# chriscoey/Hypatia.jl

Hardware: AMD Instinct MI355X
Metric: IPM iterations/sec (+ ms per KKT solve): dense n=5000, PosSemidefTri side 200 (Float64, QRCholDense + CombinedStepper) (higher is better)
Workload: dtype f64

## Files before the change

### hypatia.jl_amd/csrc/directions_multi.hip

```cpp
#include <cstring>
#include "syssolver.hpp"
#include <chrono>

namespace hyp {

void seg_dots(Ctx& c, int B, int len, const double* a, const double* b, int off, int stride, double* out);
constexpr int MR = 2;

template <int NR, int TPB, int U>
__global__ __launch_bounds__(TPB) void gemv_t_multi_kernel(int m, double alpha, const double* __restrict__ A, long lda,
                                                           const double* __restrict__ X, long ldx, double beta, double* __restrict__ Y,
                                                           long ldy) {
  constexpr int NW = TPB / 64;
  __shared__ double red[NR][NW];
  const int col = blockIdx.x;
  const double* a = A + (long)col * lda;
  double s[NR][2 * U];
#pragma unroll
  for (int r = 0; r < NR; ++r)
#pragma unroll
    for (int u = 0; u < 2 * U; ++u) s[r][u] = 0.0;
  int i = 0;
  typedef double d2_t __attribute__((ext_vector_type(2)));
  const bool wide = (((uintptr_t)a | (uintptr_t)X | ((uintptr_t)ldx * sizeof(double))) & 15) == 0;
// ... 654 lines not shown
  } else {
    for (int r = 0; r < nr; ++r) tri_solves(sol + r * ld3);
  }
  gemv_multi(ctx, false, q, n, nr, 1.0, G.d(), q, sol, ld3, 0.0, m_Gx.d(), q);
  for (size_t k = 0; k < cones.size(); ++k) {
    Cone* ck = cones[k];
    if (const int used = run_hess_prod(k, m_HGx.d() + offs[k], q, m_Gx.d() + offs[k], q, nr)) { k += used - 1; continue; }
    if (ck->use_dual_barrier) ck->inv_hess_prod(m_HGx.d() + offs[k], q, m_Gx.d() + offs[k], q, nr);
    else ck->hess_prod(m_HGx.d() + offs[k], q, m_Gx.d() + offs[k], q, nr);
  }
  {
    LinK k{};
    for (int r = 0; r < nr; ++r) { k.k0[r] = 1.0; k.k1[r] = -1.0; }
    lincomb_cols(ctx, q, nr, m_HGx.d(), q, sol + n, ld3, nullptr, 0, sol + n, ld3, k);
  }
}

void SysSolver::get_directions2(double* h_dirs, const double* h_rhss, double mu, double taubar, int max_ref_steps, double res_norm_cutoff,
                                double min_impr_tol, double* res_norms, int* n_solves) {
  HYP_REQUIRE(model_loaded, "sys: load_model first");
  const size_t d = sizeof(double);
  const int dv = dimv(), it = n + p + q, ik = dv - 1;
  *n_solves = 0;
  if (p > 0) {
    for (int r = 0; r < MR; ++r) {
      int ns = 0;
      res_norms[r] = get_directions(h_dirs + (long)r * dv, h_rhss + (long)r * dv, mu, taubar, max_ref_steps, res_norm_cutoff, min_impr_tol, &ns);
      *n_solves += ns;
    }
    return;
  }
  m_rhs.ensure((size_t)MR * dv * d);
  double* rhs = m_rhs.d();
  ctx.h2d(rhs, h_rhss, (size_t)MR * dv * d);
  Scal rs[MR], dsc[MR];
  for (int r = 0; r < MR; ++r) {
    ctx.zero(rhs + (long)r * dv + it, d);
    ctx.zero(rhs + (long)r * dv + ik, d);
    rs[r] = Scal{h_rhss[(long)r * dv + it], h_rhss[(long)r * dv + ik]};
  }
  pair_solve_device(rhs, rs, mu, taubar, max_ref_steps, res_norm_cutoff, min_impr_tol, dsc, res_norms, n_solves);
  ctx.d2h(h_dirs, m_dir.d(), (size_t)MR * dv * d);
  ctx.sync();
  for (int r = 0; r < MR; ++r) {
    h_dirs[(long)r * dv + it] = dsc[r].tau;
    h_dirs[(long)r * dv + ik] = dsc[r].kap;
  }
}

struct TauArgs { double rs_tau[2], rs_kap[2], base_tau[2], base_kap[2]; double mu, taubar, dot_const, seq; int nr, const_mode, base_on, hz_sep; };
__global__ void cols_tau_kernel(double* __restrict__ sc, TauArgs a) {
#pragma clang fp contract(off)
  if (threadIdx.x != 0) return;
  double dc = a.dot_const;
  if (a.const_mode) dc = sc[SysSolver::SC_SOLVE + 4] + (a.hz_sep ? sc[SysSolver::SC_HZ + 2] : sc[SysSolver::SC_SOLVE + 5]);
  sc[SysSolver::SC_DOTC] = dc;
  const double m2 = a.mu / a.taubar / a.taubar;
  for (int r = 0; r < a.nr; ++r) {
    const double dot_sub = sc[SysSolver::SC_SOLVE + 2 * r] + (a.hz_sep ? sc[SysSolver::SC_HZ + r] : sc[SysSolver::SC_SOLVE + 2 * r + 1]);
    const double sol_tau = (a.rs_tau[r] + a.rs_kap[r] + dot_sub) / (m2 - dc);
    const double sol_kap = -a.mu / a.taubar / a.taubar * sol_tau + a.rs_kap[r];
    sc[SysSolver::SC_CSC + 2 * r] = sol_tau;
    sc[SysSolver::SC_CSC + 2 * r + 1] = sol_kap;
    sc[SysSolver::SC_DSC + 2 * r] = a.base_on ? a.base_tau[r] - sol_tau : sol_tau;
    sc[SysSolver::SC_DSC + 2 * r + 1] = a.base_on ? a.base_kap[r] - sol_kap : sol_kap;
  }
}

struct GemvOneGuard {
  Ctx& c;
  bool keep;
  GemvOneGuard(Ctx& ctx, bool on) : c(ctx), keep(ctx.gemv_one) { if (on) c.gemv_one = true; }
  ~GemvOneGuard() { c.gemv_one = keep; }
};

void SysSolver::ensure_d_sc() {
  if (d_sc.bytes >= SC_TOTAL * sizeof(double)) return;
  d_sc.alloc(SC_TOTAL * sizeof(double));
  ctx.zero(d_sc.p, SC_TOTAL * sizeof(double));
}

static bool dir_poll_on() {
  static const bool on = [] { const char* e = getenv("HYP_DIR_POLL"); return !(e && e[0] == '0'); }();
  return on;
}

bool SysSolver::dirs_resident() const {
  static const bool on = [] { const char* e = getenv("HYP_DIR_RESIDENT"); return !(e && e[0] == '0'); }();
  static const bool dist_on = [] { const char* e = getenv("HYP_DIST_RESIDENT"); return !(e && e[0] == '0'); }();
  return on && p == 0 && (!dist() || (dist_on && fused_ok()));
}

void SysSolver::cols_solve(double* sol, const double* rhs, int nr, const Scal* rs, double mu, double taubar, bool with_const, bool joint_const,
                           bool resident, bool both, const Scal* base, Scal* dsc_host) {
  const size_t d = sizeof(double);
  const int dv = dimv();
  HYP_REQUIRE(p == 0 && nr >= 1 && nr <= MR, "cols_solve: p = 0, one or two columns");
  HYP_REQUIRE(!(with_const || joint_const) || nr == MR, "cols_solve: the constant column rides with a pair");
  const int oz = n, os = n + q + 1;
  const long ld3 = n + q;
  for (DBuf* b : {&m_subr, &m_subs}) b->ensure((size_t)(MR + 1) * ld3 * d);
  for (DBuf* b : {&m_Gx, &m_HGx, &m_Gxd}) b->ensure((size_t)(MR + 1) * q * d);
  ensure_d_sc();
  double* sr = m_subr.d();
  double* ss = m_subs.d();
  double* sc = d_sc.d();
  const int ncol = with_const ? nr + 1 : nr;
  if (with_const) {
    double* rc = const_cast<double*>(rhs) + (long)MR * dv;
    ctx.zero(rc, (size_t)dv * d);
    dev_scale_copy(ctx, n, -1.0, mc.d(), rc);
    dev_scale_copy(ctx, q, -1.0, mh.d(), rc + oz);
  }
  for (int r = 0; r < ncol; ++r) ctx.d2d(sr + r * ld3, rhs + (long)r * dv, (size_t)n * d);
  LinK neg2{};
  for (int r = 0; r < MR + 1; ++r) { neg2.k0[r] = -1.0; neg2.k1[r] = -1.0; }
  for (size_t k = 0; k < cones.size(); ++k) {
    Cone* ck = cones[k];
    const int o = offs[k], dk = ck->dim;
    if (ck->use_dual_barrier) {
      for (int r = 0; r < ncol; ++r) {
        double* tmp = ss + r * ld3 + oz + o;
        dev_scale_copy(ctx, dk, -1.0, rhs + (long)r * dv + oz + o, tmp);
        dev_axpby(ctx, dk, -1.0, rhs + (long)r * dv + os + o, 1.0, tmp);
      }
      ck->inv_hess_prod(sr + oz + o, ld3, ss + oz + o, ld3, ncol);
    } else if (const int used = run_hess_prod(k, sr + oz + o, ld3, rhs + oz + o, dv, ncol)) {
      lincomb_cols(ctx, offs[k + used] - o, ncol, sr + oz + o, ld3, rhs + os + o, dv, nullptr, 0, sr + oz + o, ld3, neg2);
      k += used - 1;
    } else {
      ck->hess_prod(sr + oz + o, ld3, rhs + oz + o, dv, ncol);
      lincomb_cols(ctx, dk, ncol, sr + oz + o, ld3, rhs + os + o, dv, nullptr, 0, sr + oz + o, ld3, neg2);
    }
  }
  {
    GemvOneGuard g1(ctx, ncol == 1);
    solve3_multi(ss, sr, ncol, joint_const ? sol_const.d() : nullptr);
  }
  const bool dist_res = resident && dist();
  {
    DotSpecs sp;
    for (int r = 0; r < ncol; ++r) {
      sp.add(n, mc.d(), ss + r * ld3, sc + SC_SOLVE + 2 * r);
      sp.add(q, mh.d(), ss + r * ld3 + oz, dist_res ? sc + SC_HZ + r : sc + SC_SOLVE + 2 * r + 1);
    }
    if (joint_const) {
      update_const_post();
      sp.add(n, mc.d(), sol_const.d(), sc + SC_SOLVE + 2 * MR);
      sp.add(q, mh.d(), sol_const.d() + n, sc + SC_SOLVE + 2 * MR + 1);
    }
    dev_dots(ctx, sp);
  }
  if (dist_res) allreduce_dev(sc + SC_HZ, ncol, 0, 2);
  const bool own_const = with_const || joint_const;
  LinK k{};
  if (resident) {
    TauArgs a{};
    for (int r = 0; r < nr; ++r) {
      a.rs_tau[r] = rs[r].tau; a.rs_kap[r] = rs[r].kap;
      if (base) { a.base_tau[r] = base[r].tau; a.base_kap[r] = base[r].kap; }
    }
    a.mu = mu; a.taubar = taubar; a.dot_const = dot_const; a.nr = nr; a.const_mode = own_const ? 1 : 0; a.base_on = base ? 1 : 0;
    a.seq = (double)(++sc_seq);
    a.hz_sep = dist_res ? 1 : 0;
    hipLaunchKernelGGL(cols_tau_kernel, dim3(1), dim3(64), 0, ctx.stream, sc, a);
    HYP_CHECK(hipGetLastError());
// ... 305 lines not shown
  double* dir = m_dir.d();
  double* res = m_res.d();
  {
    ZeroSlots z;
    for (int r = 0; r < MR; ++r) {
      z.add(dir + (long)r * dv + it); z.add(dir + (long)r * dv + ik);
      z.add(res + (long)r * dv + it); z.add(res + (long)r * dv + ik);
    }
    dev_zero_slots(ctx, z);
  }
  const bool both = (max_ref_steps > 0) && gemv_both_ok(q, n, G.d(), q);
  cols_solve(dir, rhs, MR, rs, mu, taubar, with_const, joint_const, resident, both, nullptr, dsc_host);
  if (max_ref_steps > 0) cols_residual(res, dir, rhs, MR, dsc_host, resident, false, both);
  if (read_scalars) cols_read_scalars(resident);
}

void SysSolver::pair_finish(double* rhs, const Scal* rs, double mu, double taubar, int max_ref_steps, double res_norm_cutoff,
                            double min_impr_tol, bool with_const, bool joint_const, bool resident, Scal* dsc, double* res_norms, int* n_solves) {
  const size_t d = sizeof(double);
  const int dv = dimv();
  double* dir = m_dir.d();
  double* res = m_res.d();
  const double* hp = ctx.h_sc();
  if (resident && (with_const || joint_const)) dot_const = hp[SC_DOTC];
  *n_solves += MR;
  Scal rsc[MR];
  if (max_ref_steps <= 0) {
    for (int r = 0; r < MR; ++r) {
      if (resident) dsc[r] = Scal{hp[SC_DSC + 2 * r], hp[SC_DSC + 2 * r + 1]};
      res_norms[r] = 0.0;
    }
    return;
  }
  cols_finish(MR, rs, mu, taubar, resident, dsc, rsc, res_norms);
  Gx_dir_valid = false;
  if (!(res_norms[0] > res_norm_cutoff) && !(res_norms[1] > res_norm_cutoff)) return;
  bool cones_ok = true;
  for (const Cone* ck : cones) cones_ok = cones_ok && ck->products_columnwise();
  static const bool paired = [] { const char* e = getenv("HYP_REFINE_PAIRED"); return !(e && e[0] == '0'); }();
  if (paired && cones_ok && (!dist() || resident)) {
    refine_cols(rhs, dir, res, rs, dsc, rsc, res_norms, mu, taubar, max_ref_steps, res_norm_cutoff, min_impr_tol, n_solves, resident);
    return;
  }
  for (int r = 0; r < MR; ++r) {
    if (!(res_norms[r] > res_norm_cutoff)) continue;
    double* tmp = v_tmp.d();
    ctx.d2d(tmp, dir + (long)r * dv, (size_t)dv * d);
    res_norms[r] = refine(rhs + (long)r * dv, dir + (long)r * dv, res + (long)r * dv, tmp, rs[r], dsc[r], rsc[r], res_norms[r], mu, taubar,
                          max_ref_steps, res_norm_cutoff, min_impr_tol, n_solves);
  }
}

void SysSolver::pair_solve_device(double* rhs, const Scal* rs, double mu, double taubar, int max_ref_steps, double res_norm_cutoff,
                                  double min_impr_tol, Scal* dsc, double* res_norms, int* n_solves, bool with_const, bool joint_const) {
  const bool resident = dirs_resident();
  pair_enqueue(rhs, rs, mu, taubar, max_ref_steps, with_const, joint_const, resident, dsc);
  ctx.sync();
  pair_finish(rhs, rs, mu, taubar, max_ref_steps, res_norm_cutoff, min_impr_tol, with_const, joint_const, resident, dsc, res_norms, n_solves);
}


__global__ void dder3_gate_kernel(int dk, const double* __restrict__ dots, double irtrtmu, double rteps, const double* __restrict__ D3c,
                                  const double* __restrict__ Hqp, const double* __restrict__ D3p, double* __restrict__ c0, double* __restrict__ c1) {
#pragma clang fp contract(off)
  const int k = blockIdx.y;
  const int i = blockIdx.x * blockDim.x + threadIdx.x;
  if (i >= dk) return;
  const double* dd = dots + 4 * k;
  const long e = (long)k * dk + i;
  {
    const double dot1 = dd[0], dot2 = dd[1];
    if (fabs(dot1 - dot2) / (rteps + fabs(dot2)) < 1e-4) c0[e] = D3c[e];
  }
  {
    const double dot1 = dd[2], dot2 = irtrtmu * dd[3];
    if (fabs(dot1 - dot2) / (rteps + fabs(dot2)) < 1e-4) c1[e] = Hqp[e] + D3p[e];
  }
}

void SysSolver::build_rhs_pair(int stage, double* rhs2, const double* pt, double mu, double tau, double kap, double tau_residual,
                               const double* dirs2, const double* dir_tau2, double* rs_flat, bool resident) {
  const size_t d = sizeof(double);
  const int dv = dimv(), oz = n + p, os = n + p + q + 1;
  ctx.zero(rhs2, (size_t)MR * dv * d);
  double* c0 = rhs2;
  double* c1 = rhs2 + dv;
  Scal* rs = reinterpret_cast<Scal*>(rs_flat);
  if (stage == 0) {
    const double rtmu = std::sqrt(mu);
    ctx.d2d(c1, s_resid.d(), (size_t)n * d);
    ctx.d2d(c1 + oz, s_resid.d() + n + p, (size_t)q * d);
    if (const PsdRun* r = whole_model_run()) {
      run_g.ensure((size_t)q * d);
      run_grad(*r, run_g.d());
      dev_scale_copy(ctx, q, -1.0, pt + oz, c0 + os);
      dev_axpby(ctx, q, -rtmu, run_g.d(), 1.0, c0 + os);
      dev_scale_copy(ctx, q, -1.0, pt + oz, c1 + os);
      rs[0] = Scal{0.0, -kap + mu / tau};
      rs[1] = Scal{tau_residual, -kap};
      return;
    }
    for (size_t k = 0; k < cones.size(); ++k) {
      Cone* ck = cones[k];
      const int o = offs[k], dk = ck->dim;
      const double* dual = pt + (ck->use_dual_barrier ? os : oz) + o;
      dev_scale_copy(ctx, dk, -1.0, dual, c0 + os + o);
      dev_axpby(ctx, dk, -rtmu, ck->get_grad(), 1.0, c0 + os + o);
      dev_scale_copy(ctx, dk, -1.0, dual, c1 + os + o);
    }
    rs[0] = Scal{0.0, -kap + mu / tau};
    rs[1] = Scal{tau_residual, -kap};
    return;
  }
  const double rteps = std::sqrt(2.220446049250313e-16);
  const double irtrtmu = 1.0 / std::sqrt(std::sqrt(mu));
  for (DBuf* b : {&m_Gx, &m_HGx, &m_Gxd}) b->ensure((size_t)MR * q * d);
  double* scal = m_Gx.d();
  double* Hq = m_HGx.d();
  double* D3 = m_Gxd.d();
  const size_t nc = cones.size();
  s_dots.ensure(std::max<size_t>(4 * nc, 4) * d);
  double* dots = s_dots.d();
  const PsdRun* wr = whole_model_run();
  if (wr) {
    for (int r = 0; r < MR; ++r) {
      const double* prim = dirs2 + (long)r * dv + os;
      dev_scale_copy(ctx, q, irtrtmu, prim, scal + (long)r * q);
      const int used = run_hess_prod(0, Hq + (long)r * q, q, r == 0 ? scal : prim, q, 1);
      HYP_REQUIRE(used == (int)nc, "build_rhs_pair: run product");
      run_dder3(*wr, scal + (long)r * q, D3 + (long)r * q);
      seg_dots(ctx, (int)nc, cones[0]->dim, D3 + (long)r * q, wr->point, 2 * r, 4, dots);
      seg_dots(ctx, (int)nc, cones[0]->dim, scal + (long)r * q, Hq + (long)r * q, 2 * r + 1, 4, dots);
    }
  }
  static const bool d3_paired = [] { const char* e = getenv("HYP_DDER3_PAIRED"); return !(e && e[0] == '0'); }();
  std::vector<char> done_k(nc, 0);
  for (size_t k = 0; k < nc && !wr && d3_paired; ++k) {
    PsdCone* pk = dynamic_cast<PsdCone*>(cones[k]);
    if (!pk || !pk->use_dder3() || MR != 2) continue;
    const int o = offs[k], dk = pk->dim;
    const int po = (pk->use_dual_barrier ? oz : os) + o;
    m_subs.ensure((size_t)(MR + 1) * (n + q) * d);
    double* Hin = m_subs.d();
    LinK ks{}, kh{};
    for (int r = 0; r < MR; ++r) { ks.k0[r] = irtrtmu; kh.k0[r] = (r == 0) ? irtrtmu : 1.0; }
    lincomb_cols(ctx, dk, MR, dirs2 + po, dv, nullptr, 0, nullptr, 0, scal + o, q, ks);
    lincomb_cols(ctx, dk, MR, dirs2 + po, dv, nullptr, 0, nullptr, 0, Hin, dk, kh);
    pk->hess_prod_slow(Hq + o, q, Hin, dk, MR);
    pk->dder3_cols(scal + o, q, MR, D3 + o, q);
    done_k[k] = 1;
  }
  for (size_t k = 0; k < nc && !wr; ++k) {
    Cone* ck = cones[k];
    if (!ck->use_dder3() || done_k[k]) continue;
    const int o = offs[k], dk = ck->dim;
    const int po = (ck->use_dual_barrier ? oz : os) + o;
    for (int r = 0; r < MR; ++r) {
      const double* prim = dirs2 + (long)r * dv + po;
      double* sc = scal + (long)r * q + o;
      double* hh = Hq + (long)r * q + o;
      dev_scale_copy(ctx, dk, irtrtmu, prim, sc);
      ck->hess_prod_slow(hh, q, r == 0 ? sc : prim, q, 1);
      const double* d3 = ck->dder3(sc);
      ctx.d2d(D3 + (long)r * q + o, d3, (size_t)dk * d);
    }
  }
  for (size_t k = 0; k < nc && !wr; ++k) {
    Cone* ck = cones[k];
    if (!ck->use_dder3()) continue;
    const int o = offs[k], dk = ck->dim;
    if (d3_paired) {
      DotSpecs sp;
      for (int r = 0; r < MR; ++r) {
        sp.add(dk, D3 + (long)r * q + o, ck->point.d(), dots + 4 * k + 2 * r);
        sp.add(dk, scal + (long)r * q + o, Hq + (long)r * q + o, dots + 4 * k + 2 * r + 1);
      }
      dev_dots(ctx, sp);
      continue;
    }
    for (int r = 0; r < MR; ++r) {
      dev_dot(ctx, dk, D3 + (long)r * q + o, ck->point.d(), dots + 4 * k + 2 * r);
      dev_dot(ctx, dk, scal + (long)r * q + o, Hq + (long)r * q + o, dots + 4 * k + 2 * r + 1);
    }
  }
  const double tc = dir_tau2[0] / tau, tp = dir_tau2[1] / tau;
  rs[0] = Scal{0.0, tc * mu / tau * tc};
  rs[1] = Scal{0.0, tp * mu / tau * (1.0 + tp)};
  if (resident) {
    if (wr) {
      const int dk = cones[0]->dim;
      hipLaunchKernelGGL(dder3_gate_kernel, dim3((dk + 255) / 256, (unsigned)nc), dim3(256), 0, ctx.stream, dk, dots, irtrtmu, rteps, D3, Hq + q,
                         D3 + q, c0 + os, c1 + os);
    } else {
      for (size_t k = 0; k < nc; ++k) {
        Cone* ck = cones[k];
        if (!ck->use_dder3()) continue;
        const int o = offs[k], dk = ck->dim;
        hipLaunchKernelGGL(dder3_gate_kernel, dim3((dk + 255) / 256, 1), dim3(256), 0, ctx.stream, dk, dots + 4 * k, irtrtmu, rteps, D3 + o,
                           Hq + q + o, D3 + q + o, c0 + os + o, c1 + os + o);
      }
    }
    HYP_CHECK(hipGetLastError());
    return;
  }
  std::vector<double> hd(4 * std::max<size_t>(nc, 1));
  ctx.d2h(hd.data(), dots, 4 * nc * d);
  ctx.sync();
  for (size_t k = 0; k < nc; ++k) {
    Cone* ck = cones[k];
    if (!ck->use_dder3()) continue;
    const int o = offs[k], dk = ck->dim;
    {
      const double dot1 = hd[4 * k], dot2 = hd[4 * k + 1];
      if (std::fabs(dot1 - dot2) / (rteps + std::fabs(dot2)) < 1e-4) ctx.d2d(c0 + os + o, D3 + o, (size_t)dk * d);
    }
    {
      const double dot1 = hd[4 * k + 2], dot2 = irtrtmu * hd[4 * k + 3];
      if (std::fabs(dot1 - dot2) / (rteps + std::fabs(dot2)) < 1e-4) {
        ctx.d2d(c1 + os + o, Hq + q + o, (size_t)dk * d);
        dev_axpby(ctx, dk, 1.0, D3 + q + o, 1.0, c1 + os + o);
      }
    }
  }
}

void SysSolver::step_directions(const double* h_point, const double* h_res, double tau_residual, double mu, int max_ref_steps,
                                double res_norm_cutoff, double min_impr_tol, double* h_dirs, double* res_norms, int* n_solves,
                                int* use_sqrt_out, int* info, int* used_fallback, double* h_sol_const) {
  HYP_REQUIRE(model_loaded, "sys: load_model first");
  HYP_REQUIRE(p == 0, "step_directions: p = 0 only");
  const size_t d = sizeof(double);
  const int dv = dimv(), it = n + p + q, ik = dv - 1;
  *n_solves = 0;
  *info = 0;
  *used_fallback = 0;
  s_resident = false;
  double* hs_point = ctx.stage_host((size_t)dv + 2 * (size_t)it + 2 * (size_t)MR * dv);
  double* hs_res = hs_point + dv;
  double* hs_const = hs_res + it;
  double* hs_dirs = hs_const + it;
  s_point.ensure((size_t)dv * d);
  s_resid.ensure((size_t)it * d);
  auto upload = [&](hipStream_t st) {
    std::memcpy(hs_point, h_point, (size_t)dv * d);
    std::memcpy(hs_res, h_res, (size_t)it * d);
    HYP_CHECK(hipMemcpyAsync(s_point.p, hs_point, (size_t)dv * d, hipMemcpyHostToDevice, st));
    HYP_CHECK(hipMemcpyAsync(s_resid.p, hs_res, (size_t)it * d, hipMemcpyHostToDevice, st));
  };
  const bool resident_flow = dirs_resident() && nmp > 0 && !getenv_on("HYP_FORCE_BK") && !getenv_on("HYP_FORCE_FACT_FAIL");
  static const bool late_upload = [] { const char* e = getenv("HYP_LATE_UPLOAD"); return !(e && e[0] == '0'); }();
  const bool upload_late = resident_flow && late_upload && ctx.stream == ctx.stream_primary && (size_t)dv * d >= (1u << 20);
  if (upload_late) {
    if (!up_ev0) {
      HYP_CHECK(hipEventCreateWithFlags(&up_ev0, hipEventDisableTiming));
      HYP_CHECK(hipEventCreateWithFlags(&up_ev1, hipEventDisableTiming));
    }
    HYP_CHECK(hipEventRecord(up_ev0, ctx.stream));
  }
  static const bool after_env = [] { const char* e = getenv("HYP_UPLOAD_AFTER"); return !(e && e[0] == '0'); }();
  const bool upload_after = resident_flow && !upload_late && after_env;
  if (!upload_late && !upload_after) upload(ctx.stream);
  const auto t0 = std::chrono::steady_clock::now();
  const double tau = h_point[it], kap = h_point[ik];
  m_rhs.ensure((size_t)(MR + 1) * dv * d);
  v_tmp.ensure((size_t)MR * dv * d);
  const bool resident = resident_flow;
  if (!resident) {
    if (nmp > 0) update_lhs_fact(info, used_fallback);
    if (use_sqrt_out)
      for (size_t k = 0; k < cones.size(); ++k) use_sqrt_out[k] = use_sqrt[k];
    if (*info != 0) { ctx.sync(); return; }
    step_directions_rest(false, tau, kap, tau_residual, mu, max_ref_steps, res_norm_cutoff, min_impr_tol, h_dirs, res_norms, n_solves,
                         h_sol_const, hs_const, hs_dirs, false, nullptr, nullptr);
    last_update_lhs_s = last_rest_update_lhs_s + std::chrono::duration<double>(t_rest0 - t0).count();
    return;
  }
  assemble_lhs();
  factor_lhs_begin();
  if (upload_after) {
    hs_point = ctx.stage_host((size_t)dv + 2 * (size_t)it + 2 * (size_t)MR * dv);
    hs_res = hs_point + dv;
    hs_const = hs_res + it;
    hs_dirs = hs_const + it;
    upload(ctx.stream);
  }
  if (upload_late) {
    hs_point = ctx.stage_host((size_t)dv + 2 * (size_t)it + 2 * (size_t)MR * dv);
    hs_res = hs_point + dv;
    hs_const = hs_res + it;
    hs_dirs = hs_const + it;
    HYP_CHECK(hipStreamWaitEvent(ctx.stream2, up_ev0, 0));
    upload(ctx.stream2);
    HYP_CHECK(hipEventRecord(up_ev1, ctx.stream2));
    HYP_CHECK(hipStreamWaitEvent(ctx.stream, up_ev1, 0));
  }
  if (use_sqrt_out)
    for (size_t k = 0; k < cones.size(); ++k) use_sqrt_out[k] = use_sqrt[k];
  bool cones_ok = true;
  for (const Cone* ck : cones) cones_ok = cones_ok && ck->products_columnwise();
  const bool const3 = const3_on() && cones_ok;
  const bool joint = !const3 && tri3_on() && !dist() && tri.ready(nmp) && tri.sb > 0 && tri.sb <= 1024;
  if (!const3 && !joint) {
    update_const();
    if (h_sol_const) ctx.d2h(hs_const, sol_const.p, (size_t)it * d);
  }
  if (joint) update_const_pre();
  HYP_CHECK(hipEventRecord(ctx.ev[5], ctx.stream));
  Scal rs[MR], dsc[MR];
  double rn[MR];
  int ns = 0;
  build_rhs_pair(0, m_rhs.d(), s_point.d(), mu, tau, kap, tau_residual, nullptr, nullptr, reinterpret_cast<double*>(rs), true);
  pair_enqueue(m_rhs.d(), rs, mu, tau, max_ref_steps, const3, joint, true, dsc);
  wait_scalars();
  if (dir_poll_on() && ctx.h_sc_dev != nullptr) ctx.h_info[Ctx::H_INFO_FACT] = (int)ctx.h_sc()[SC_INFO];
  const auto tf0 = std::chrono::steady_clock::now();
  factor_lhs_end(info, used_fallback, true);
  const double fallback_s = std::chrono::duration<double>(std::chrono::steady_clock::now() - tf0).count();
  auto read_times = [&] {
    factor_lhs_times();
    float ms = 0;
    HYP_CHECK(hipEventElapsedTime(&ms, ctx.ev[0], ctx.ev[5]));
    last_update_lhs_s = 1e-3 * ms;
  };
  if (*info != 0 || use_bk) read_times();
  if (*info != 0) return;
  if (use_bk) {
    const double dev_s = last_update_lhs_s;
    step_directions_rest(false, tau, kap, tau_residual, mu, max_ref_steps, res_norm_cutoff, min_impr_tol, h_dirs, res_norms, n_solves,
                         h_sol_const, hs_const, hs_dirs, false, nullptr, nullptr);
    last_update_lhs_s = dev_s + fallback_s + last_rest_update_lhs_s;
    return;
  }
  pair_finish(m_rhs.d(), rs, mu, tau, max_ref_steps, res_norm_cutoff, min_impr_tol, const3, joint, true, dsc, rn, &ns);
  if ((const3 || joint) && h_sol_const) ctx.d2h(hs_const, sol_const.p, (size_t)it * d);
  *n_solves += ns;
  step_directions_rest(true, tau, kap, tau_residual, mu, max_ref_steps, res_norm_cutoff, min_impr_tol, h_dirs, res_norms, n_solves, h_sol_const,
                       hs_const, hs_dirs, true, dsc, rn);
  read_times();
}

static bool env_default_on(const char* name) {
  const char* e = getenv(name);
  return !(e && e[0] == '0');
}
bool SysSolver::const3_on() { static const bool on = env_default_on("HYP_CONST_COL3"); return on; }
bool SysSolver::tri3_on() { static const bool on = env_default_on("HYP_CONST_TRI3"); return on; }
bool SysSolver::getenv_on(const char* name) {
  const char* e = getenv(name);
  return e && e[0] && e[0] != '0';
}

void SysSolver::step_directions_rest(bool resident, double tau, double kap, double tau_residual, double mu, int max_ref_steps,
                                     double res_norm_cutoff, double min_impr_tol, double* h_dirs, double* res_norms, int* n_solves,
                                     double* h_sol_const, double* hs_const, double* hs_dirs, bool first_pair_done, Scal* d01_in, double* rn01) {
  const size_t d = sizeof(double);
  const int dv = dimv(), it = n + p + q, ik = dv - 1;
  t_rest0 = std::chrono::steady_clock::now();
  last_rest_update_lhs_s = 0.0;
  Scal rs[MR], dsc[MR];
  double rn[MR];
  int ns = 0;
  if (!first_pair_done) {
    bool cones_ok = true;
    for (const Cone* ck : cones) cones_ok = cones_ok && ck->products_columnwise();
    const bool const3 = const3_on() && !use_bk && cones_ok;
    const bool joint = !const3 && tri3_on() && !dist() && !use_bk && nmp > 0 && tri.ready(nmp) && tri.sb > 0 && tri.sb <= 1024;
    if (!const3 && !joint) {
      update_const();
      if (h_sol_const) ctx.d2h(hs_const, sol_const.p, (size_t)it * d);
    }
    if (joint) update_const_pre();
    last_rest_update_lhs_s = std::chrono::duration<double>(std::chrono::steady_clock::now() - t_rest0).count();
    build_rhs_pair(0, m_rhs.d(), s_point.d(), mu, tau, kap, tau_residual, nullptr, nullptr, reinterpret_cast<double*>(rs), resident);
    pair_enqueue(m_rhs.d(), rs, mu, tau, max_ref_steps, const3, joint, resident, dsc);
    ctx.sync();
    pair_finish(m_rhs.d(), rs, mu, tau, max_ref_steps, res_norm_cutoff, min_impr_tol, const3, joint, resident, dsc, rn, &ns);
    if ((const3 || joint) && h_sol_const) ctx.d2h(hs_const, sol_const.p, (size_t)it * d);
    *n_solves += ns;
  } else {
    dsc[0] = d01_in[0]; dsc[1] = d01_in[1];
    rn[0] = rn01[0]; rn[1] = rn01[1];
  }
  res_norms[0] = rn[0];
  res_norms[1] = rn[1];
  s_dirs.ensure((size_t)2 * MR * dv * d);
  const double dtau[MR] = {dsc[0].tau, dsc[1].tau};
  const Scal d01[MR] = {dsc[0], dsc[1]};
  build_rhs_pair(1, m_rhs.d(), s_point.d(), mu, tau, kap, tau_residual, m_dir.d(), dtau, reinterpret_cast<double*>(rs), resident);
  const size_t rows_down = dirs_x_only ? (size_t)n : (size_t)dv;
  auto dirs_d2h = [&](int half) {
    double* dst = hs_dirs + (long)half * MR * dv;
    if (!dirs_x_only) { ctx.d2h(dst, m_dir.d(), (size_t)MR * dv * d); return; }
    HYP_CHECK(hipMemcpy2DAsync(dst, (size_t)dv * d, m_dir.d(), (size_t)dv * d, rows_down * d, MR, hipMemcpyDeviceToHost, ctx.stream));
  };
  auto dirs_out = [&](int half) {
    for (int r = 0; r < MR; ++r)
      std::memcpy(h_dirs + ((long)half * MR + r) * dv, hs_dirs + ((long)half * MR + r) * dv, rows_down * d);
  };
  dirs_d2h(0);
  ctx.d2d(s_dirs.p, m_dir.p, (size_t)MR * dv * d);
  if (!dirs_copied_ev) HYP_CHECK(hipEventCreateWithFlags(&dirs_copied_ev, hipEventDisableTiming));
  HYP_CHECK(hipEventRecord(dirs_copied_ev, ctx.stream));
  ns = 0;
  pair_enqueue(m_rhs.d(), rs, mu, tau, max_ref_steps, false, false, resident, dsc, false);
  dirs_d2h(1);
  ctx.d2d(s_dirs.d() + (long)MR * dv, m_dir.p, (size_t)MR * dv * d);
  cols_read_scalars(resident);
  HYP_CHECK(hipEventSynchronize(dirs_copied_ev));
  dirs_out(0);
  if (resident) wait_scalars();
  else ctx.sync();
  const int ns_before = ns;
  pair_finish(m_rhs.d(), rs, mu, tau, max_ref_steps, res_norm_cutoff, min_impr_tol, false, false, resident, dsc, rn, &ns);
  *n_solves += ns;
  res_norms[2] = rn[0];
  res_norms[3] = rn[1];
  if (ns > ns_before + MR) {
    dirs_d2h(1);
    ctx.d2d(s_dirs.d() + (long)MR * dv, m_dir.p, (size_t)MR * dv * d);
    ctx.sync();
  }
  dirs_out(1);
  if (h_sol_const) std::memcpy(h_sol_const, hs_const, (size_t)it * d);
  for (int r = 0; r < MR; ++r) {
    h_dirs[(long)r * dv + it] = d01[r].tau;
    h_dirs[(long)r * dv + ik] = d01[r].kap;
    h_dirs[(long)(MR + r) * dv + it] = dsc[r].tau;
    h_dirs[(long)(MR + r) * dv + ik] = dsc[r].kap;
    s_tk[1 + r][0] = d01[r].tau;
    s_tk[1 + r][1] = d01[r].kap;
    s_tk[1 + MR + r][0] = dsc[r].tau;
    s_tk[1 + MR + r][1] = dsc[r].kap;
  }
  s_tk[0][0] = tau;
  s_tk[0][1] = kap;
  s_resident_q = q;
  s_resident = (MR == 2);
}

}
```

### hypatia.jl_amd/csrc/syssolver.hpp

```cpp
#pragma once
#include <chrono>
#include "cones.hpp"

namespace hyp {

void dev_sub_absmax(Ctx& c, int n, double* a, const double* b, double* d_out);
void dev_sub_absmax_cols(Ctx& c, int n, int nr, double* a, const double* b, long ld, double* d_out, double* work);

struct SysSolver {
  Ctx& ctx;
  int n, p, q, nmp;
  std::vector<Cone*> cones;
  std::vector<int> offs;
  DBuf G;
  DBuf GQ1;
  DBuf GQ2s;
  DBuf Qm;
  DBuf Rinv;
  DBuf HGQ2;
  DBuf lhs;
  DBuf lhs_tri;
  DBuf lhs_fact, dinv, d_info;
  TriSolvePlan tri;
  DBuf QpbxGHbz, Gx, HGx, GQ1x, HGQ1x, tmpn, sol, rhs, tmpq;
// ... 77 lines not shown
  void allreduce_fused(double* d_buf, long npay, const FusedTail& t, double* h_out, int site);
  void allreduce_fused_dev(double* d_buf, long npay, const FusedTail& t, int site);
  double screen_sz_[18];
  double screen_szfail_[18];
  int screen_pass_g_ = -1;
  DBuf rp_x, rp_z, rp_s, rp_t, rp_g;
  DBuf rp_loc;
  void prefetch_residual_products(int mode, double alpha, const double* d_cand, const double* h_cand);
  bool rp_pre_valid = false;
  double* rp_pre_host = nullptr;
  size_t rp_pre_host_n = 0;
  hipEvent_t rp_pre_ev = nullptr;
  std::vector<double> rp_pre_cand;
  long rp_pre_hits = 0, rp_pre_misses = 0;
  void residual_products2(const double* h_x, const double* h_z, const double* h_s, double tau, double* h_Gtz, double* h_Gx_s, double* h_dots,
                          double* h_norms);
  void residual_products(const double* h_x, const double* h_z, const double* h_s, double* h_Gtz, double* h_Gx_s, double* h_dots);

  DBuf mc, mb, mh, mA;
  DBuf v_rhs, v_dir, v_res, v_tmp;
  DBuf sub_rhs, sub_sol, sol_const;
  bool model_loaded = false;
  double dot_const = 0.0;
  DBuf Gx_dir;
  bool Gx_dir_valid = false;
  int dimv() const { return n + p + q + 1 + q + 1; }
  void load_model(const double* hc, const double* hb, const double* hh, const double* hA);
  void sgemv(bool trans, int m, int n_, double alpha, const double* A, long lda, const double* x, double beta, double* y);
  void update_const();
  void update_const_pre();
  void update_const_post();
  struct Scal { double tau, kap; };
  Scal solve_system(double* d_sol, const double* d_rhs, Scal rhs, double mu, double taubar);
  Scal apply_lhs(double* d_res, const double* d_dir, Scal dir, double mu, double taubar);
  DBuf cand_d;
  bool check_cone_points(const double* h_ztsk, double min_prox, double prox_bound, bool use_max_prox, double nup1, double* prox_out,
                         int* n_loaded, double* irtmu_out);
  static constexpr int SCREEN_MAX = 18;
  DBuf screen_buf, screen_info;
  long screen_count = 0, screen_rejected = 0;
  int gprev_acc_ = -1;
  long screen_checked = 0, screen_mismatch = 0;
  bool cand_scalars(const double* h, double min_prox, double prox_bound, double nup1, double* irtmu) const;
  bool screen_usable() const { return screen_mode() != 0; }
  int screen_agreed = -1;
  int screen_kmax() const;
  int screen_mode() const;
  void screen_candidates_run(const double* d_cands, int K, const double* tau, const double* kap, double min_prox, double prox_bound,
                             double nup1, bool use_max_prox, char* rej);
  bool screen_survivor = false;
  void screen_candidates(const double* d_cands, int K, const double* tau, const double* kap, double min_prox, double prox_bound, double nup1,
                         char* rej);
  bool s_resident = false;
  int s_resident_q = -1;
  double s_tk[5][2] = {{0, 0}, {0, 0}, {0, 0}, {0, 0}, {0, 0}};
  double residual(double* res, const double* dir, const double* rhs, Scal rs, Scal dcur, Scal& rsc, double mu, double taubar);
  double residual_fused(double* res, const double* dir, const double* rhs, Scal rs, Scal dcur, Scal& rsc, double mu, double taubar);
  DBuf rf_buf;
  double refine(double* rhs, double* dir, double* res, double* tmp, Scal rs, Scal& dsc, Scal rsc, double res_norm, double mu, double taubar,
                int max_ref_steps, double res_norm_cutoff, double min_impr_tol, int* n_solves);
  DBuf m_rhs, m_dir, m_res, m_subr, m_subs, m_t, m_Gx, m_HGx, m_Gxd;
  void solve3_multi(double* sol, const double* rhs, int nr, double* x_third = nullptr);
  void get_directions2(double* h_dirs, const double* h_rhss, double mu, double taubar, int max_ref_steps, double res_norm_cutoff,
                       double min_impr_tol, double* res_norms, int* n_solves);
  int search_alpha(const double* pt, const double* d_cent, const double* d_pred, const double* d_centadj, const double* d_predadj,
                   bool unadj_only, bool cent_only, const double* sched, int nsched, int start, double min_prox, double prox_bound,
                   bool use_max_prox, double nup1, double* cand_out, double* prox_out, int* n_trials, int* n_loaded, double* irtmu_out,
                   bool resident = false);
  DBuf s_point, s_resid, s_dots, s_dirs;
  double last_update_lhs_s = 0.0;
  void build_rhs_pair(int stage, double* rhs2, const double* d_point, double mu, double tau, double kap, double tau_residual,
                      const double* d_dirs2, const double* dir_tau2, double* rs_flat , bool resident = false);
  void step_directions(const double* h_point, const double* h_res, double tau_residual, double mu, int max_ref_steps,
                       double res_norm_cutoff, double min_impr_tol, double* h_dirs, double* res_norms, int* n_solves, int* use_sqrt_out,
                       int* info, int* used_fallback, double* h_sol_const);
  void pair_solve_device(double* rhs2, const Scal* rs, double mu, double taubar, int max_ref_steps, double res_norm_cutoff,
                         double min_impr_tol, Scal* dsc, double* res_norms, int* n_solves, bool with_const = false, bool joint_const = false);
  DBuf d_sc;
  enum { SC_SOLVE = 0, SC_RESD = 8, SC_AMAX = 12, SC_DSC = 16, SC_DOTC = 20, SC_HZ = 21, SC_CSC = 24, SC_INFO = 30, SC_SEQ = 31, SC_N = 32, SC_WORK = 64, SC_TOTAL = 64 + 3 * 33 + 5 };
  unsigned long sc_seq = 0;
  void wait_scalars();
  void ensure_d_sc();
  bool dirs_resident() const;
  void cols_solve(double* sol, const double* rhs, int nr, const Scal* rs, double mu, double taubar, bool with_const, bool joint_const,
                  bool resident, bool both, const Scal* base, Scal* dsc_host);
  void cols_residual(double* res, const double* dir, const double* rhs, int nr, const Scal* dsc_host, bool resident, bool fresh, bool both);
  void cols_read_scalars(bool resident);
  void cols_finish(int nr, const Scal* rs, double mu, double taubar, bool resident, Scal* dsc, Scal* rsc, double* res_norms);
  void refine_cols(double* rhs, double* dir, double* res, const Scal* rs, Scal* dsc, Scal* rsc, double* res_norms, double mu, double taubar,
                   int max_ref_steps, double res_norm_cutoff, double min_impr_tol, int* n_solves, bool resident);
  void pair_enqueue(double* rhs2, const Scal* rs, double mu, double taubar, int max_ref_steps, bool with_const, bool joint_const,
                    bool resident, Scal* dsc_host, bool read_scalars = true);
  void pair_finish(double* rhs2, const Scal* rs, double mu, double taubar, int max_ref_steps, double res_norm_cutoff, double min_impr_tol,
                   bool with_const, bool joint_const, bool resident, Scal* dsc, double* res_norms, int* n_solves);
  static bool const3_on();
  static bool tri3_on();
  static bool getenv_on(const char* name);
  bool dirs_x_only = false;
  hipEvent_t up_ev0 = nullptr, up_ev1 = nullptr;
  hipEvent_t dirs_copied_ev = nullptr;
  std::chrono::steady_clock::time_point t_rest0;
  double last_rest_update_lhs_s = 0.0;
  void step_directions_rest(bool resident, double tau, double kap, double tau_residual, double mu, int max_ref_steps, double res_norm_cutoff,
                            double min_impr_tol, double* h_dirs, double* res_norms, int* n_solves, double* h_sol_const, double* hs_const,
                            double* hs_dirs, bool first_pair_done, Scal* d01, double* rn01);
  double get_directions(double* h_dir, const double* h_rhs, double mu, double taubar, int max_ref_steps, double res_norm_cutoff,
                        double min_impr_tol, int* n_solves);
};

struct SymIndefSys {
  Ctx& ctx;
  int n, p, q, npq;
  std::vector<Cone*> cones;
  std::vector<int> offs;
  DBuf lhs;
  DBuf fact, dinv, xb;
  BKFact bk;
  TriSolvePlan tri;
  bool fact_ok = false;
  SymIndefSys(Ctx& c, int n_, int p_, int q_, const std::vector<Cone*>& cs);
  void load(const double* hA, const double* hG);
  void update_lhs(int* info, int* used_fallback);
  void solve3(double* h_sol, const double* h_rhs);
};

}
```

### hypatia.jl_amd/csrc/gemm_f64_kernel.hpp

```cpp
#pragma once
#include "gemm_f64.hpp"
#include <vector>

namespace hyp {

#ifdef HYP_GEMM_PROBE
__device__ unsigned long long gemm_probe_acc[8];
#define GEMM_PROBE_T(x) const unsigned long long x = __builtin_amdgcn_s_memtime()
#else
#define GEMM_PROBE_T(x)
#endif

constexpr int BK = 16, LDS_S = BK + 2;
typedef const volatile double __attribute__((address_space(3))) lds_cv_f64;
constexpr int GEMM_THREADS = 256;

__device__ __forceinline__ void upper_tile_from_linear(int idx, int& tm, int& tn) {
  int t = (int)((sqrt(8.0 * (double)idx + 1.0) - 1.0) * 0.5);
  while ((long)(t + 1) * (t + 2) / 2 <= idx) ++t;
  while ((long)t * (t + 1) / 2 > idx) --t;
  tn = t;
  tm = idx - t * (t + 1) / 2;
}

// ... 84 lines not shown
      rb[2 * rep] = tb.x; rb[2 * rep + 1] = tb.y;
    }
  };
  auto store_tiles_fast = [&](int buf) {
    double* As = lds[buf][0];
    double* Bs = lds[buf][1];
#pragma unroll
    for (int rep = 0; rep < REPS2; ++rep) {
      *reinterpret_cast<d2_t*>(As + (vr + 32 * rep) * LDS_S + vk) = (d2_t){ra[2 * rep], ra[2 * rep + 1]};
      *reinterpret_cast<d2_t*>(Bs + (vr + 32 * rep) * LDS_S + vk) = (d2_t){rb[2 * rep], rb[2 * rep + 1]};
    }
  };

  auto load_tiles = [&](int k0) {
    if (fast && k0 + BK <= kend) {
      load_tiles_fast(k0);
      return;
    }

    const int klast = kend - 1;
    if (TRANSA) {
      const int kc = min(k0 + lk, klast);
#pragma unroll
      for (int rep = 0; rep < REPS; ++rep) ra[rep] = A[(long)min(m0 + lr + 16 * rep, p.M - 1) * p.lda + kc];
    } else {
      const int mc = min(m0 + nn_r, p.M - 1);
#pragma unroll
      for (int rep = 0; rep < REPS; ++rep) ra[rep] = A[(long)min(k0 + nn_k + NN_KSTEP * rep, klast) * p.lda + mc];
    }
    {
      const int kc = min(k0 + lk, klast);
#pragma unroll
      for (int rep = 0; rep < REPS; ++rep) rb[rep] = B[(long)min(n0 + lr + 16 * rep, p.N - 1) * p.ldb + kc];
    }
  };

  auto store_tiles = [&](int buf, int k0) {
    if (fast && k0 + BK <= kend) {
      store_tiles_fast(buf);
      return;
    }
    double* As = lds[buf][0];
    double* Bs = lds[buf][1];
    const double kmask = (k0 + lk < kend) ? 1.0 : 0.0;
    if (TRANSA) {
#pragma unroll
      for (int rep = 0; rep < REPS; ++rep) As[(lr + 16 * rep) * LDS_S + lk] = ra[rep] * ((m0 + lr + 16 * rep < p.M) ? kmask : 0.0);
    } else {
      const double mmask = (m0 + nn_r < p.M) ? 1.0 : 0.0;
#pragma unroll
      for (int rep = 0; rep < REPS; ++rep)
        As[nn_r * LDS_S + nn_k + NN_KSTEP * rep] = ra[rep] * ((k0 + nn_k + NN_KSTEP * rep < kend) ? mmask : 0.0);
    }
#pragma unroll
    for (int rep = 0; rep < REPS; ++rep) Bs[(lr + 16 * rep) * LDS_S + lk] = rb[rep] * ((n0 + lr + 16 * rep < p.N) ? kmask : 0.0);
  };

  const int fr = lane & 15, fk = lane >> 4;

  auto compute = [&](int buf) {
    const double* As = lds[buf][0] + (wm * WT + fr) * LDS_S + fk;
    const double* Bs = lds[buf][1] + (wn * WT + fr) * LDS_S + fk;
#pragma unroll
    for (int kk = 0; kk < BK; kk += 4) {
      double af[TW], bf[TW];
#pragma unroll
#ifdef HYP_GEMM_READ2
      for (int i = 0; i < TW; ++i) af[i] = As[i * 16 * LDS_S + kk];
#pragma unroll
      for (int j = 0; j < TW; ++j) bf[j] = Bs[j * 16 * LDS_S + kk];
#else
      for (int i = 0; i < TW; ++i) af[i] = *(lds_cv_f64*)(As + i * 16 * LDS_S + kk);
#pragma unroll
      for (int j = 0; j < TW; ++j) bf[j] = *(lds_cv_f64*)(Bs + j * 16 * LDS_S + kk);
#endif
#pragma unroll
      for (int j = 0; j < TW; ++j)
#pragma unroll
        for (int i = 0; i < TW; ++i)
          acc[j][i] = __builtin_amdgcn_mfma_f64_16x16x4f64(bf[j], af[i], acc[j][i], 0, 0, 0);
    }
  };

  const int nkt = (kend > kbeg) ? (kend - kbeg + BK - 1) / BK : 0;
#ifdef HYP_GEMM_PROBE
  unsigned long long pr_req = 0, pr_mma = 0, pr_sto = 0, pr_bar = 0;
  GEMM_PROBE_T(pr_birth);
#endif
  if (nkt > 0) {
    load_tiles(kbeg);
    store_tiles(0, kbeg);
    __syncthreads();
    for (int t = 0; t < nkt; ++t) {
      const int buf = t & 1;
      GEMM_PROBE_T(c0);
      if (t + 1 < nkt) load_tiles(kbeg + (t + 1) * BK);
      GEMM_PROBE_T(c1);
      compute(buf);
      GEMM_PROBE_T(c2);
      if (t + 1 < nkt) store_tiles(buf ^ 1, kbeg + (t + 1) * BK);
      GEMM_PROBE_T(c3);
      __syncthreads();
#ifdef HYP_GEMM_PROBE
      const unsigned long long c4 = __builtin_amdgcn_s_memtime();
      pr_req += c1 - c0; pr_mma += c2 - c1; pr_sto += c3 - c2; pr_bar += c4 - c3;
#endif
    }
  }
#ifdef HYP_GEMM_PROBE
  if (lane == 0) {
    atomicAdd(&gemm_probe_acc[0], pr_req); atomicAdd(&gemm_probe_acc[1], pr_mma); atomicAdd(&gemm_probe_acc[2], pr_sto);
    atomicAdd(&gemm_probe_acc[3], pr_bar); atomicAdd(&gemm_probe_acc[4], (unsigned long long)nkt); atomicAdd(&gemm_probe_acc[5], 1ull);
    atomicAdd(&gemm_probe_acc[6], __builtin_amdgcn_s_memtime() - pr_birth);
  }
#endif

  const bool upper = (p.tri != GEMM_FULL);
  if (p.splitk > 1) {
    double* __restrict__ W = p.part + ((long)bz * p.splitk + blockIdx.z) * p.part_stride;
    if (TAG == 1 && p.tile_cnt != nullptr) {
#pragma unroll
      for (int j = 0; j < TW; ++j)
#pragma unroll
        for (int r = 0; r < 4; ++r) {
          const int n = n0 + wn * WT + j * 16 + fk + 4 * r;
          if (n >= p.N) continue;
#pragma unroll
          for (int i = 0; i < TW; ++i) {
            const int m = m0 + wm * WT + i * 16 + fr;
            if (m >= p.M || (upper && m > n + p.tri_off)) continue;
            __hip_atomic_store(&W[(long)n * p.part_ld + m], acc[j][i][r], __ATOMIC_RELAXED, __HIP_MEMORY_SCOPE_AGENT);
          }
        }
      asm volatile("s_waitcnt vmcnt(0)" ::: "memory");
      __shared__ int last_in;
      __syncthreads();
      if (tid == 0) {
        const int expect = (p.tail_q > 1 && (int)blockIdx.x >= p.tail_first) ? p.splitk_base - 1 + p.tail_q : p.splitk_base;
        const int old = __hip_atomic_fetch_add(&p.tile_cnt[blockIdx.x], 1, __ATOMIC_RELAXED, __HIP_MEMORY_SCOPE_AGENT);
        last_in = (old == expect - 1) ? 1 : 0;
        if (last_in) __hip_atomic_store(&p.tile_cnt[blockIdx.x], 0, __ATOMIC_RELAXED, __HIP_MEMORY_SCOPE_AGENT);
      }
      __syncthreads();
      if (!last_in) return;
      const int S = p.splitk_base;
      const int S_extra = (p.tail_q > 1 && (int)blockIdx.x >= p.tail_first) ? p.tail_q - 1 : 0;
      const double* __restrict__ P0 = p.part + (long)bz * p.splitk * p.part_stride;
#pragma unroll
      for (int j = 0; j < TW; ++j)
#pragma unroll
        for (int r = 0; r < 4; ++r) {
          const int n = n0 + wn * WT + j * 16 + fk + 4 * r;
          if (n >= p.N) continue;
#pragma unroll
          for (int i = 0; i < TW; ++i) {
            const int m = m0 + wm * WT + i * 16 + fr;
            if (m >= p.M || (upper && m > n + p.tri_off)) continue;
            const long off = (long)n * p.part_ld + m;
            double s = 0.0;
            for (int z = 0; z < S + S_extra; ++z) s += __hip_atomic_load(&P0[(long)z * p.part_stride + off], __ATOMIC_RELAXED, __HIP_MEMORY_SCOPE_AGENT);
            double* cp = C + (long)n * p.ldc + m;
            *cp = p.alpha * s + (p.beta != 0.0 ? p.beta * (*cp) : 0.0);
          }
        }
      return;
    }
#pragma unroll
    for (int j = 0; j < TW; ++j)
#pragma unroll
      for (int r = 0; r < 4; ++r) {
        const int n = n0 + wn * WT + j * 16 + fk + 4 * r;
        if (n >= p.N) continue;
#pragma unroll
        for (int i = 0; i < TW; ++i) {
          const int m = m0 + wm * WT + i * 16 + fr;
          if (m >= p.M || (upper && m > n + p.tri_off)) continue;
          W[(long)n * p.part_ld + m] = acc[j][i][r];
        }
      }
    return;
  }
  if (p.beta != 0.0 && p.cm_blk == 0) {
#pragma unroll
    for (int j = 0; j < TW; ++j) {
      double cold[4][TW];
#pragma unroll
      for (int r = 0; r < 4; ++r) {
        const int nc = min(n0 + wn * WT + j * 16 + fk + 4 * r, p.N - 1);
#pragma unroll
        for (int i = 0; i < TW; ++i) cold[r][i] = C[(long)nc * p.ldc + min(m0 + wm * WT + i * 16 + fr, p.M - 1)];
      }
#pragma unroll
      for (int r = 0; r < 4; ++r)
#pragma unroll
        for (int i = 0; i < TW; ++i) asm volatile("" : "+v"(cold[r][i]));
// ... 389 lines not shown
```

Baseline: 57.76.

## Enqueue stage-1 RHS build before host wait so it overlaps factorization

For PSD-only, non-distributed problems, the stage-1 (corrector) right-hand side is now built on the device into a separate buffer right after the first pair is enqueued and before the host waits on scalars. Later, if refinement did not take extra solves, only the host-side tau scalars are computed and the device rebuild is skipped. The goal is to hide the RHS-building kernels and their launch latency behind the host wait. The cost is an extra buffer, more state flags, and a dependence on m_dir being final when the early build runs. A stale flag forces a rebuild when refinement ran more solves.

```diff
diff --git a/hypatia.jl_amd/csrc/directions_multi.hip b/hypatia.jl_amd/csrc/directions_multi.hip
--- a/hypatia.jl_amd/csrc/directions_multi.hip
+++ b/hypatia.jl_amd/csrc/directions_multi.hip
@@ -760,6 +760,11 @@
 
 static bool dir_poll_on() {
   static const bool on = [] { const char* e = getenv("HYP_DIR_POLL"); return !(e && e[0] == '0'); }();
+  return on;
+}
+
+bool SysSolver::dir_fuse_on() {
+  static const bool on = [] { const char* e = getenv("HYP_DIR_FUSE"); return !(e && e[0] == '0'); }();
   return on;
 }
 
@@ -1231,6 +1236,13 @@
                                const double* dirs2, const double* dir_tau2, double* rs_flat, bool resident) {
   const size_t d = sizeof(double);
   const int dv = dimv(), oz = n + p, os = n + p + q + 1;
+  auto stage1_scalars = [&] {
+    Scal* rs1 = reinterpret_cast<Scal*>(rs_flat);
+    const double tc = dir_tau2[0] / tau, tp = dir_tau2[1] / tau;
+    rs1[0] = Scal{0.0, tc * mu / tau * tc};
+    rs1[1] = Scal{0.0, tp * mu / tau * (1.0 + tp)};
+  };
+  if (stage == 1 && !rhs2) { stage1_scalars(); return; }
   ctx.zero(rhs2, (size_t)MR * dv * d);
   double* c0 = rhs2;
   double* c1 = rhs2 + dv;
@@ -1332,9 +1344,8 @@
       dev_dot(ctx, dk, scal + (long)r * q + o, Hq + (long)r * q + o, dots + 4 * k + 2 * r + 1);
     }
   }
-  const double tc = dir_tau2[0] / tau, tp = dir_tau2[1] / tau;
-  rs[0] = Scal{0.0, tc * mu / tau * tc};
-  rs[1] = Scal{0.0, tp * mu / tau * (1.0 + tp)};
+  HYP_REQUIRE(dir_tau2 || resident, "build_rhs_pair: the device work alone needs the acceptance tests on the device");
+  if (dir_tau2) stage1_scalars();
   if (resident) {
     if (wr) {
       const int dk = cones[0]->dim;
@@ -1460,6 +1471,16 @@
   int ns = 0;
   build_rhs_pair(0, m_rhs.d(), s_point.d(), mu, tau, kap, tau_residual, nullptr, nullptr, reinterpret_cast<double*>(rs), true);
   pair_enqueue(m_rhs.d(), rs, mu, tau, max_ref_steps, const3, joint, true, dsc);
+  stage1_queued = false;
+  if (dir_fuse_on() && !dist()) {
+    bool psd_only = true;
+    for (Cone* ck : cones) psd_only = psd_only && dynamic_cast<PsdCone*>(ck) != nullptr;
+    if (psd_only) {
+      m_rhs1.ensure((size_t)MR * dv * d);
+      build_rhs_pair(1, m_rhs1.d(), s_point.d(), mu, tau, kap, tau_residual, m_dir.d(), nullptr, nullptr, true);
+      stage1_queued = true;
+    }
+  }
   wait_scalars();
   if (dir_poll_on() && ctx.h_sc_dev != nullptr) ctx.h_info[Ctx::H_INFO_FACT] = (int)ctx.h_sc()[SC_INFO];
   const auto tf0 = std::chrono::steady_clock::now();
@@ -1483,6 +1504,7 @@
   pair_finish(m_rhs.d(), rs, mu, tau, max_ref_steps, res_norm_cutoff, min_impr_tol, const3, joint, true, dsc, rn, &ns);
   if ((const3 || joint) && h_sol_const) ctx.d2h(hs_const, sol_const.p, (size_t)it * d);
   *n_solves += ns;
+  stage1_stale = ns > MR;
   step_directions_rest(true, tau, kap, tau_residual, mu, max_ref_steps, res_norm_cutoff, min_impr_tol, h_dirs, res_norms, n_solves, h_sol_const,
                        hs_const, hs_dirs, true, dsc, rn);
   read_times();
@@ -1535,7 +1557,11 @@
   s_dirs.ensure((size_t)2 * MR * dv * d);
   const double dtau[MR] = {dsc[0].tau, dsc[1].tau};
   const Scal d01[MR] = {dsc[0], dsc[1]};
-  build_rhs_pair(1, m_rhs.d(), s_point.d(), mu, tau, kap, tau_residual, m_dir.d(), dtau, reinterpret_cast<double*>(rs), resident);
+  const bool early = first_pair_done && resident && stage1_queued;
+  stage1_queued = false;
+  double* rhs1 = early ? m_rhs1.d() : m_rhs.d();
+  build_rhs_pair(1, (early && !stage1_stale) ? nullptr : rhs1, s_point.d(), mu, tau, kap, tau_residual, m_dir.d(), dtau,
+                 reinterpret_cast<double*>(rs), resident);
   const size_t rows_down = dirs_x_only ? (size_t)n : (size_t)dv;
   auto dirs_d2h = [&](int half) {
     double* dst = hs_dirs + (long)half * MR * dv;
@@ -1551,7 +1577,7 @@
   if (!dirs_copied_ev) HYP_CHECK(hipEventCreateWithFlags(&dirs_copied_ev, hipEventDisableTiming));
   HYP_CHECK(hipEventRecord(dirs_copied_ev, ctx.stream));
   ns = 0;
-  pair_enqueue(m_rhs.d(), rs, mu, tau, max_ref_steps, false, false, resident, dsc, false);
+  pair_enqueue(rhs1, rs, mu, tau, max_ref_steps, false, false, resident, dsc, false);
   dirs_d2h(1);
   ctx.d2d(s_dirs.d() + (long)MR * dv, m_dir.p, (size_t)MR * dv * d);
   cols_read_scalars(resident);
@@ -1560,7 +1586,7 @@
   if (resident) wait_scalars();
   else ctx.sync();
   const int ns_before = ns;
-  pair_finish(m_rhs.d(), rs, mu, tau, max_ref_steps, res_norm_cutoff, min_impr_tol, false, false, resident, dsc, rn, &ns);
+  pair_finish(rhs1, rs, mu, tau, max_ref_steps, res_norm_cutoff, min_impr_tol, false, false, resident, dsc, rn, &ns);
   *n_solves += ns;
   res_norms[2] = rn[0];
   res_norms[3] = rn[1];
diff --git a/hypatia.jl_amd/csrc/syssolver.hpp b/hypatia.jl_amd/csrc/syssolver.hpp
--- a/hypatia.jl_amd/csrc/syssolver.hpp
+++ b/hypatia.jl_amd/csrc/syssolver.hpp
@@ -183,6 +183,10 @@
   void wait_scalars();
   void ensure_d_sc();
   bool dirs_resident() const;
+  static bool dir_fuse_on();
+  DBuf m_rhs1;
+  bool stage1_queued = false;
+  bool stage1_stale = false;
   void cols_solve(double* sol, const double* rhs, int nr, const Scal* rs, double mu, double taubar, bool with_const, bool joint_const,
                   bool resident, bool both, const Scal* base, Scal* dsc_host);
   void cols_residual(double* res, const double* dir, const double* rhs, int nr, const Scal* dsc_host, bool resident, bool fresh, bool both);
```

Result: no change. 58.08, median of 5 (+0.5%).

## Add software-pipelined interior K loop with interleaved global loads for TRANSA GEMM

Applied to the files above, without the earlier changes.

Adds a fast path for the transposed-A, TW=4, TAG=1 GEMM variant when the full K range is interior and offsets fit in 32 bits. Global loads are issued two K-tiles ahead into register sets, and LDS stores and loads are interleaved between individual MFMA groups under scheduling barriers. The LDS fragments are double-buffered across the k-substeps. The aim is to hide global-memory and LDS latency behind MFMA work and replace __syncthreads with a lighter waitcnt plus barrier. Remaining tail tiles fall back to the generic loop. Costs are higher register pressure and complexity, and stale-load clamping at k_last adds redundant loads.

```diff
diff --git a/hypatia.jl_amd/csrc/gemm_f64_kernel.hpp b/hypatia.jl_amd/csrc/gemm_f64_kernel.hpp
--- a/hypatia.jl_amd/csrc/gemm_f64_kernel.hpp
+++ b/hypatia.jl_amd/csrc/gemm_f64_kernel.hpp
@@ -190,23 +190,111 @@
     }
   };
 
-  const int nkt = (kend > kbeg) ? (kend - kbeg + BK - 1) / BK : 0;
 #ifdef HYP_GEMM_PROBE
   unsigned long long pr_req = 0, pr_mma = 0, pr_sto = 0, pr_bar = 0;
   GEMM_PROBE_T(pr_birth);
 #endif
+  int kgen = kbeg;
+  if constexpr (TRANSA && TW == 4 && TAG == 1) {
+    const bool interior = fast && p.krange == KR_ALL && (kend - kbeg) >= 2 * BK && (long)BM * p.lda < (1L << 28) && (long)BN * p.ldb < (1L << 28);
+    if (interior) {
+      const int nfull = (kend - kbeg) / BK;
+      const int k_last = kbeg + (nfull - 1) * BK;
+      const char* ga = reinterpret_cast<const char*>(A + (long)m0 * p.lda);
+      const char* gb = reinterpret_cast<const char*>(B + (long)n0 * p.ldb);
+      unsigned offa[REPS2], offb[REPS2];
+#pragma unroll
+      for (int rep = 0; rep < REPS2; ++rep) {
+        offa[rep] = (unsigned)(((long)(vr + 32 * rep) * p.lda + vk) * 8);
+        offb[rep] = (unsigned)(((long)(vr + 32 * rep) * p.ldb + vk) * 8);
+      }
+      d2_t sa[2][REPS2], sb[2][REPS2];
+      auto request = [&](int set, int r, int k0) {
+        unsigned o = (r & 1) ? offb[r >> 1] : offa[r >> 1];
+        asm("" : "+v"(o) : "s"(k0));
+        if (r & 1) sb[set][r >> 1] = *reinterpret_cast<const d2_t*>(gb + (long)k0 * 8 + o);
+        else sa[set][r >> 1] = *reinterpret_cast<const d2_t*>(ga + (long)k0 * 8 + o);
+      };
+      auto store_one = [&](int set, int r, int buf) {
+        if (r & 1) *reinterpret_cast<d2_t*>(lds[buf][1] + (vr + 32 * (r >> 1)) * LDS_S + vk) = sb[set][r >> 1];
+        else *reinterpret_cast<d2_t*>(lds[buf][0] + (vr + 32 * (r >> 1)) * LDS_S + vk) = sa[set][r >> 1];
+      };
+      auto phase = [&](int buf, bool stage, int set, int k_req) {
+        GEMM_PROBE_T(c1);
+        const double* As = lds[buf][0] + (wm * WT + fr) * LDS_S + fk;
+        const double* Bs = lds[buf][1] + (wn * WT + fr) * LDS_S + fk;
+        double af[2][TW], bf[2][TW];
+#pragma unroll
+        for (int i = 0; i < TW; ++i) af[0][i] = *(lds_cv_f64*)(As + i * 16 * LDS_S);
+#pragma unroll
+        for (int j = 0; j < TW; ++j) bf[0][j] = *(lds_cv_f64*)(Bs + j * 16 * LDS_S);
+#pragma unroll
+        for (int s = 0; s < BK / 4; ++s) {
+          const int cur = s & 1, nxt = cur ^ 1;
+#pragma unroll
+          for (int j = 0; j < TW; ++j) {
+#pragma unroll
+            for (int i = 0; i < TW; ++i)
+              acc[j][i] = __builtin_amdgcn_mfma_f64_16x16x4f64(bf[cur][j], af[cur][i], acc[j][i], 0, 0, 0);
+            if (stage && s * TW + j < 2 * REPS2) {
+              store_one(set, s * TW + j, buf ^ 1);
+              request(set, s * TW + j, min(k_req, k_last));
+            }
+            if (s + 1 < BK / 4 && j == 0) {
+#pragma unroll
+              for (int i = 0; i < TW; ++i) af[nxt][i] = *(lds_cv_f64*)(As + i * 16 * LDS_S + 4 * (s + 1));
+            }
+            if (s + 1 < BK / 4 && j == 1) {
+#pragma unroll
+              for (int jj = 0; jj < TW; ++jj) bf[nxt][jj] = *(lds_cv_f64*)(Bs + jj * 16 * LDS_S + 4 * (s + 1));
+            }
+            __builtin_amdgcn_sched_barrier(0);
+          }
+        }
+        GEMM_PROBE_T(c2);
+        asm volatile("s_waitcnt lgkmcnt(0)" ::: "memory");
+        __builtin_amdgcn_s_barrier();
+        asm volatile("" ::: "memory");
+        __builtin_amdgcn_sched_barrier(0);
+#ifdef HYP_GEMM_PROBE
+        const unsigned long long c3 = __builtin_amdgcn_s_memtime();
+        pr_mma += c2 - c1; pr_bar += c3 - c2;
+#endif
+      };
+#pragma unroll
+      for (int r = 0; r < 2 * REPS2; ++r) request(0, r, kbeg);
+#pragma unroll
+      for (int r = 0; r < 2 * REPS2; ++r) store_one(0, r, 0);
+#pragma unroll
+      for (int r = 0; r < 2 * REPS2; ++r) request(1, r, kbeg + BK);
+#pragma unroll
+      for (int r = 0; r < 2 * REPS2; ++r) request(0, r, min(kbeg + 2 * BK, k_last));
+      asm volatile("s_waitcnt lgkmcnt(0)" ::: "memory");
+      __builtin_amdgcn_s_barrier();
+      asm volatile("" ::: "memory");
+      __builtin_amdgcn_sched_barrier(0);
+      int k0 = kbeg;
+      for (; k0 < k_last; k0 += 2 * BK) {
+        phase(0, true, 1, k0 + 3 * BK);
+        phase(1, true, 0, k0 + 4 * BK);
+      }
+      if (k0 == k_last) phase(0, false, 0, 0);
+      kgen = kbeg + nfull * BK;
+    }
+  }
+  const int nkt = (kend > kgen) ? (kend - kgen + BK - 1) / BK : 0;
   if (nkt > 0) {
-    load_tiles(kbeg);
-    store_tiles(0, kbeg);
+    load_tiles(kgen);
+    store_tiles(0, kgen);
     __syncthreads();
     for (int t = 0; t < nkt; ++t) {
       const int buf = t & 1;
       GEMM_PROBE_T(c0);
-      if (t + 1 < nkt) load_tiles(kbeg + (t + 1) * BK);
+      if (t + 1 < nkt) load_tiles(kgen + (t + 1) * BK);
       GEMM_PROBE_T(c1);
       compute(buf);
       GEMM_PROBE_T(c2);
-      if (t + 1 < nkt) store_tiles(buf ^ 1, kbeg + (t + 1) * BK);
+      if (t + 1 < nkt) store_tiles(buf ^ 1, kgen + (t + 1) * BK);
       GEMM_PROBE_T(c3);
       __syncthreads();
 #ifdef HYP_GEMM_PROBE
@@ -218,7 +306,7 @@
 #ifdef HYP_GEMM_PROBE
   if (lane == 0) {
     atomicAdd(&gemm_probe_acc[0], pr_req); atomicAdd(&gemm_probe_acc[1], pr_mma); atomicAdd(&gemm_probe_acc[2], pr_sto);
-    atomicAdd(&gemm_probe_acc[3], pr_bar); atomicAdd(&gemm_probe_acc[4], (unsigned long long)nkt); atomicAdd(&gemm_probe_acc[5], 1ull);
+    atomicAdd(&gemm_probe_acc[3], pr_bar); atomicAdd(&gemm_probe_acc[4], (unsigned long long)(nkt + (kgen - kbeg) / BK)); atomicAdd(&gemm_probe_acc[5], 1ull);
     atomicAdd(&gemm_probe_acc[6], __builtin_amdgcn_s_memtime() - pr_birth);
   }
 #endif
```

After: 56.94 before, 55.29 after. -2.9%, worse.
